# zju3dv/object_nerf

Hardware: NVIDIA H100
Metric: rays/s (higher is better)
Workload: dtype bf16

## Files before the change

object_nerf_b200/csrc/field_tc.cu:

```cuda
#include <cuda_bf16.h>

#include "encode.cuh"
#include "field_common.cuh"
#include "tc_chain.cuh"
#include "field_pe.cuh"
#include "prune.cuh"

namespace {

using namespace tc;

constexpr float kLeaky = 0.01f;

enum Epi { EPI_HIDDEN = 0, EPI_HIDDEN_RC = 1, EPI_HIDDEN_SIGMA = 2, EPI_FINAL = 3, EPI_DIR = 4 };

struct TcParams {
  FieldParams f;
  WLayer layers[MAX_LAYERS];
  int n_layers;
  uint8_t* dump;
  TrainLayout TL;
  uint32_t* diag;
#ifdef ONERF_FIELD_TIMELINE
  uint64_t* tl;
#endif
};

struct RowMeta {
  int ray, si, mute, live;
};

struct Rows {
  int row[2];
  int live[2];
  int ray[2], si[2], mute[2];
  const float* rc[2];
  int64_t tile;
#ifdef ONERF_FIELD_TIMELINE
  uint64_t* tl;
#endif
};

__device__ __forceinline__ void fragment_rows(int (&row)[2], int warp, int lane) {
  row[0] = (warp >> 2) * 64 + (warp & 3) * 16 + (lane >> 2);
  row[1] = row[0] + 8;
}

#ifdef ONERF_FIELD_TIMELINE
constexpr int TL_CTAS = 8, TL_TILES = 16, TL_SLOTS = 80;
uint64_t* g_timeline = nullptr;
__device__ __forceinline__ void tl_put(uint64_t* tl, int slot, uint64_t v) {
  asm volatile("{\n\t.reg .pred p;\n\tsetp.ne.u64 p, %0, 0;\n\t@p st.global.u64 [%1], %2;\n\t}" ::"l"(tl), "l"(tl + slot),
               "l"(v)
               : "memory");
}
__device__ __forceinline__ uint64_t* tl_record(const TcParams& P, int64_t tile, int wg, bool lead) {
  const int64_t k = (tile - blockIdx.x) / gridDim.x;
  if (!P.tl || !lead || blockIdx.x >= TL_CTAS || k >= TL_TILES) return nullptr;
  return P.tl + (((int64_t)blockIdx.x * 3 + wg) * TL_TILES + k) * TL_SLOTS;
}
#define TL_AT(tl, slot) tl_put((tl), (slot), clock64())
#define TL_PUT(tl, slot, v) tl_put((tl), (slot), (v))
#else
#define TL_AT(tl, slot)
#define TL_PUT(tl, slot, v)
#endif

__device__ __forceinline__ uint32_t leaky_bf16x2(uint32_t x) {
  __nv_bfloat162 v = *reinterpret_cast<__nv_bfloat162*>(&x);
  const __nv_bfloat162 slope = __floats2bfloat162_rn(kLeaky, kLeaky);
  v = __hmax2(v, __hmul2(v, slope));
  return *reinterpret_cast<uint32_t*>(&v);
}

template <int N>
__device__ __forceinline__ void dump_layer(const TcParams& P, const Rows& R, int slot, int mask_word0, const uint32_t* pk) {
  const int q = threadIdx.x & 3;
#pragma unroll
  for (int r = 0; r < 2; ++r) {
    const int row = R.row[r];
    uint8_t* base = P.dump + P.TL.act_off[slot] + ((size_t)R.tile * P.TL.act_atoms[slot]) * ATOM_BYTES + (size_t)row * 128 + q * 4;
#pragma unroll
    for (int j = 0; j < N / 8; ++j)
      *reinterpret_cast<uint32_t*>(base + (size_t)(j >> 3) * ATOM_BYTES + (((j & 7) ^ (row & 7)) << 4)) = pk[2 * j + r];
  }
  if (mask_word0 < 0) return;
  constexpr int CPW = N >= 128 ? 32 : 16, NW = N / CPW, BPW = CPW / 8;
  uint32_t* mrow = reinterpret_cast<uint32_t*>(P.dump + P.TL.mask_off) + ((size_t)R.tile * ONERF_MASK_WORDS + mask_word0) * 128;
#pragma unroll
  for (int w = 0; w < NW; ++w) {
#pragma unroll
    for (int r = 0; r < 2; ++r) {
      uint32_t m = 0;
#pragma unroll
      for (int jj = 0; jj < BPW; ++jj) {
        const uint32_t v = pk[2 * (w * BPW + jj) + r];
        const uint32_t bits = (((v >> 15) & 1u) ^ 1u) | ((((v >> 31) & 1u) ^ 1u) << 1);
        m |= bits << (8 * jj + 2 * q);
      }
      m |= __shfl_xor_sync(0xffffffffu, m, 1);
      m |= __shfl_xor_sync(0xffffffffu, m, 2);
      if (q == 0) mrow[w * 128 + R.row[r]] = m;
    }
  }
}

template <int N, int EPI>
__device__ __forceinline__ void epilogue(const float (&acc)[N / 2], uint32_t* pk, const float* bias, const Rows& R,
                                         int rc_base, const float* headw, float (&part)[2][4]) {
  const int q = threadIdx.x & 3;
#pragma unroll
  for (int j = 0; j < N / 8; ++j) {
    const int c = 8 * j + 2 * q;
    float2 b[2];
    if (EPI == EPI_HIDDEN_RC || EPI == EPI_DIR) {
      b[0] = __ldg(reinterpret_cast<const float2*>(R.rc[0] + rc_base + c));
      b[1] = __ldg(reinterpret_cast<const float2*>(R.rc[1] + rc_base + c));
    } else {
      b[0] = b[1] = *reinterpret_cast<const float2*>(bias + c);
    }
#pragma unroll
    for (int r = 0; r < 2; ++r) {
      float t0 = acc[4 * j + 2 * r] + b[r].x, t1 = acc[4 * j + 2 * r + 1] + b[r].y;
      uint32_t p;
      if (EPI == EPI_HIDDEN || EPI == EPI_HIDDEN_RC) {
        p = leaky_bf16x2(pack_bf16(t0, t1));
      } else if (EPI == EPI_FINAL) {
        p = pack_bf16(t0, t1);
      } else {
        t0 = fmaxf(t0, t0 * kLeaky);
        t1 = fmaxf(t1, t1 * kLeaky);
        if (EPI == EPI_HIDDEN_SIGMA) {
          const float2 w = __ldg(reinterpret_cast<const float2*>(headw + c));
          part[r][0] = fmaf(t1, w.y, fmaf(t0, w.x, part[r][0]));
        } else {
#pragma unroll
          for (int k = 0; k < 3; ++k) {
            const float2 w = __ldg(reinterpret_cast<const float2*>(headw + k * N + c));
            part[r][1 + k] = fmaf(t1, w.y, fmaf(t0, w.x, part[r][1 + k]));
          }
        }
        p = pack_bf16(t0, t1);
      }
      pk[2 * j + r] = p;
    }
  }
}

__device__ __forceinline__ float row_sum(float part) {
  part += __shfl_xor_sync(0xffffffffu, part, 1);
  part += __shfl_xor_sync(0xffffffffu, part, 2);
  return part;
}

__device__ __forceinline__ void write_heads(const FieldParams& p, const Rows& R, int branch, float (&part)[2][4],
                                            float* outp) {
  const float* Pf = reinterpret_cast<const float*>(p.packed);
  const float* hb = Pf + (branch ? p.L.orgb_b : p.L.rgb_b);
  const float sb = __ldg(Pf + (branch ? p.L.osigma_b : p.L.sigma_b));
#pragma unroll
  for (int r = 0; r < 2; ++r) {
#pragma unroll
    for (int k = 0; k < 4; ++k) part[r][k] = row_sum(part[r][k]);
    if ((threadIdx.x & 3) == 0 && R.live[r]) {
      float sg = part[r][0] + sb;
      const float cr = 1.0f / (1.0f + __expf(-(part[r][1] + __ldg(hb + 0))));
      const float cg = 1.0f / (1.0f + __expf(-(part[r][2] + __ldg(hb + 1))));
      const float cb = 1.0f / (1.0f + __expf(-(part[r][3] + __ldg(hb + 2))));
      if (R.mute[r] & (branch ? 2 : 1)) sg = -1e5f;
      reinterpret_cast<float4*>(outp)[(int64_t)R.ray[r] * p.out_stride + R.si[r]] = make_float4(cr, cg, cb, sg);
    }
  }
}

__device__ __forceinline__ void x_release(uint32_t x_free, bool on) {
  asm volatile(
      "{\n\t.reg .pred p;\n\tsetp.eq.u32 p, %1, 1;\n\t@p mbarrier.arrive.shared::cta.b64 _, [%0];\n\t}" ::"r"(x_free),
      "r"((uint32_t)on & (uint32_t)((threadIdx.x & 31) == 0))
      : "memory");
}

template <int N, int NX, int NH, int EPI, bool DUMP>
__device__ __forceinline__ void run_layer(const TcParams& P, const Rows& R, Ring& ring, uint32_t sXw, float (&acc)[N / 2],
                                          const uint32_t* hin, uint32_t* hout, const float* bias, int rc_base,
                                          const float* headw, float (&part)[2][4], int slot, int mask_word0,
                                          uint32_t x_free = 0, bool free_x = false) {
  TL_AT(R.tl, 3 * slot);
  mma_layer<N, NX, NH>(acc, hin, sXw, ring);
  if constexpr (NX > 0) x_release(x_free, free_x);
  TL_AT(R.tl, 3 * slot + 1);
#ifdef ONERF_FIELD_TIMELINE
  TL_PUT(R.tl, 55 + slot, ring.full_wait);
  ring.full_wait = 0;
#endif
  epilogue<N, EPI>(acc, hout, bias, R, rc_base, headw, part);
  if (DUMP) dump_layer<N>(P, R, slot, mask_word0, hout);
  TL_AT(R.tl, 3 * slot + 2);
}

template <int XS, bool DUMP>
__device__ __forceinline__ void scene_trunk(const TcParams& P, const Rows& R, Ring& ring, uint32_t sXw, float (&acc)[128],
                                            uint32_t (&h)[64], const float* bias_tab, float (&part)[2][4],
                                            uint32_t x_free) {
  const float* sw = reinterpret_cast<const float*>(P.f.packed) + P.f.L.sigma_w;
  run_layer<256, XS, 0, EPI_HIDDEN, DUMP>(P, R, ring, sXw, acc, h, h, bias_tab + G_S0 * 256, 0, nullptr, part, 1,
                                          onerf_mask_word0(1), x_free, false);
#pragma unroll 1
  for (int l = 1; l < 4; ++l)
    run_layer<256, 0, 8, EPI_HIDDEN, DUMP>(P, R, ring, sXw, acc, h, h, bias_tab + (G_S0 + l) * 256, 0, nullptr, part,
                                           1 + l, onerf_mask_word0(1 + l));
  run_layer<256, XS, 8, EPI_HIDDEN, DUMP>(P, R, ring, sXw, acc, h, h, bias_tab + G_S4 * 256, 0, nullptr, part, 5,
                                          onerf_mask_word0(5), x_free, true);
#pragma unroll 1
  for (int l = 5; l < 7; ++l)
    run_layer<256, 0, 8, EPI_HIDDEN, DUMP>(P, R, ring, sXw, acc, h, h, bias_tab + (G_S0 + l) * 256, 0, nullptr, part,
                                           1 + l, onerf_mask_word0(1 + l));
  run_layer<256, 0, 8, EPI_HIDDEN_SIGMA, DUMP>(P, R, ring, sXw, acc, h, h, bias_tab + G_S7 * 256, 0, sw, part, 8,
                                               onerf_mask_word0(8));
}

constexpr int NUM_ENCODER = 3 * 32;

__device__ __forceinline__ void prefetch_l2(const void* ptr) {
  asm volatile("prefetch.global.L2 [%0];" ::"l"(ptr));
}

__device__ __forceinline__ void prefetch_rows(const void* base, int64_t pitch, int64_t bytes0, int nbytes, int r0,
                                              int r1, int et) {
  const int lines = (nbytes + 127) >> 7;
  for (int i = et; i < (r1 - r0 + 1) * lines; i += NUM_ENCODER)
    prefetch_l2(reinterpret_cast<const char*>(base) + (r0 + i / lines) * pitch + bytes0 + (int64_t)(i % lines) * 128);
}

__device__ __forceinline__ void voxel_encode_job(const GridView& g, uint32_t sX, int row, int cq, float x, float y,
                                                 float z, uint32_t x_free, uint32_t parity, uint32_t* diag) {
  if (cq < 3) {
    float f[8];
    if (cq == 0) voxel_trilinear<0, 8, false>(g, x, y, z, f);
    else if (cq == 1) voxel_trilinear<8, 8, false>(g, x, y, z, f);
    else voxel_trilinear<16, 8, false>(g, x, y, z, f);
    mbar_wait(x_free, parity, diag);
    pe8_to_chunks(sX, row, cq < 2 ? cq : 34, cq < 2 ? 2 : 1, f);
  } else if (cq == 3) {
    mbar_wait(x_free, parity, diag);
    pe_xyz_to_chunks(sX, row, 26, x, y, z);
    st_chunk(a_chunk_addr(sX, row, 47), 0u, 0u, 0u, 0u);
  }
}

template <bool VOXEL>
__device__ __forceinline__ void encoder_loop(const TcParams& P, uint32_t sX, RowMeta* meta, uint32_t x_full,
                                             uint32_t x_free, int64_t n_tiles, int64_t total) {
  const FieldParams& p = P.f;
  const int et = threadIdx.x - NUM_CONSUMER - 32;
  constexpr int JOBS = VOXEL ? 4 * TM : TM;
  uint32_t it = 0;
  for (int64_t tile = blockIdx.x; tile < n_tiles; tile += gridDim.x, ++it) {
#ifdef ONERF_FIELD_TIMELINE
    uint64_t* tl = tl_record(P, tile, 2, et == 0);
#endif
    TL_AT(tl, 0);
    {
      const int64_t e0 = tile * TM, e1 = min(e0 + TM, total) - 1;
      prefetch_rows(p.ray_const, ONERF_RAY_CONST_FLOATS * 4, 0, ONERF_RAY_CONST_FLOATS * 4, (int)(e0 / p.S),
                    (int)(e1 / p.S), et);
      const int64_t n0 = e0 + (int64_t)gridDim.x * TM, n1 = min(n0 + TM, total) - 1;
      if (n0 < total) {
        prefetch_rows(p.rays, 32, 0, 32, (int)(n0 / p.S), (int)(n1 / p.S), et);
        prefetch_rows(p.z, p.z_stride * 4, 0, p.S * 4, (int)(n0 / p.S), (int)(n1 / p.S), et);
      }
    }
#pragma unroll 1
    for (int job = et; job < JOBS; job += NUM_ENCODER) {
      const int row = job & (TM - 1), cq = job / TM;
      const int64_t e = tile * TM + row;
      const bool live = e < total;
      const int ray = live ? (int)(e / p.S) : 0;
      const int si = live ? (int)(e - (int64_t)ray * p.S) : 0;
      const float* rr = p.rays + (int64_t)ray * 8;
      const float zz = live ? __ldg(p.z + (int64_t)ray * p.z_stride + si) : 0.0f;
      float x = fmaf(__ldg(rr + 3), zz, __ldg(rr + 0));
      float y = fmaf(__ldg(rr + 4), zz, __ldg(rr + 1));
      float z = fmaf(__ldg(rr + 5), zz, __ldg(rr + 2));
      if (p.xyz && live) {
        const float* qq = p.xyz + ((int64_t)ray * p.S + si) * 3;
        x = __ldg(qq); y = __ldg(qq + 1); z = __ldg(qq + 2);
      }
      if (!live) { x = 0.f; y = 0.f; z = 0.f; }
      if (cq == 0) {
        int mute = 0;
        if (live && p.mute_zero_rays && __ldg(p.z + (int64_t)ray * p.z_stride + (p.S - 1)) == 0.0f) mute = 3;
        if (live && mute == 0 && p.n_boxes > 0 && point_in_boxes(p.boxes, p.n_boxes, x, y, z)) mute = 1;
        mbar_wait(x_free, (it & 1) ^ 1, P.diag);
        meta[row] = RowMeta{ray, si, mute, live ? 1 : 0};
      }
      if (VOXEL) {
        voxel_encode_job(load_grid_view(p.grid), sX, row, cq, x, y, z, x_free, (it & 1) ^ 1, P.diag);
      } else if (cq == 0) {
        mbar_wait(x_free, (it & 1) ^ 1, P.diag);
        pe_xyz_to_chunks(sX, row, 0, x, y, z);
      }
    }
    mbar_wait(x_free, (it & 1) ^ 1, P.diag);
    TL_AT(tl, 1);
    fence_async_smem();
    mbar_arrive(x_full);
    TL_AT(tl, 2);
  }
}

struct FieldSmem {
  uint32_t sB, sBias, sMeta, sBar, x_full, x_free, bytes;
};
__host__ __device__ constexpr FieldSmem field_smem(int x_atoms, bool has_meta) {
  FieldSmem s{};
  s.sB = x_atoms * ATOM_BYTES;
  s.sBias = s.sB + NSTAGE * STAGE_BYTES;
  s.sMeta = s.sBias + G_COUNT * 256 * 4;
  s.sBar = s.sMeta + (has_meta ? TM * (uint32_t)sizeof(RowMeta) : 0u);
  s.x_full = s.sBar + 16 * NSTAGE;
  s.x_free = s.x_full + 8;
  s.bytes = 1024 + s.x_free + 8;
  return s;
}

__device__ __forceinline__ Ring cta_prologue(const FieldSmem& S, const TcParams& P, uint32_t sX, float* bias_tab) {
  const FieldParams& p = P.f;
  const float* Pf = reinterpret_cast<const float*>(p.packed);
  Ring ring{sX + S.sB, sX + S.sBar, sX + S.sBar + 8 * NSTAGE, 0u, 0u, P.diag};
  if (threadIdx.x == 0) {
    mbar_init(sX + S.x_full, NUM_ENCODER);
    mbar_init(sX + S.x_free, NUM_CONSUMER / 32);
    ring_init_bars(ring.full, ring.empty);
  }
  for (int i = threadIdx.x; i < G_COUNT * 256; i += NUM_THREADS) {
    const int g = i >> 8, c = i & 255;
    bias_tab[i] = (c < p.L.g[g].N) ? __ldg(Pf + p.L.g[g].bias_off + c) : 0.0f;
  }
  __syncthreads();
  return ring;
}

struct CodeLoop {
  int n;
  int64_t rc_stride, obj_stride;
};

template <bool VOXEL, bool DUMP, bool MULTI>
__device__ __forceinline__ void field_tc_body(const TcParams& P, const CodeLoop& cl) {
  extern __shared__ __align__(1024) uint8_t smem_raw[];
  const FieldParams& p = P.f;
  const int warp = threadIdx.x >> 5, lane = threadIdx.x & 31;
  constexpr int X_ATOMS = VOXEL ? 6 : 1;
  constexpr int XS = VOXEL ? 9 : 2, XO = VOXEL ? 12 : 2;
  constexpr FieldSmem S = field_smem(X_ATOMS, true);
  const uint32_t sX = (smem_u32(smem_raw) + 1023u) & ~1023u;
  uint8_t* gen_base = smem_raw + (sX - smem_u32(smem_raw));
  float* bias_tab = reinterpret_cast<float*>(gen_base + S.sBias);
  RowMeta* meta = reinterpret_cast<RowMeta*>(gen_base + S.sMeta);
  const uint32_t x_full = sX + S.x_full, x_free = sX + S.x_free;
  const float* Pf = reinterpret_cast<const float*>(p.packed);
  Ring ring = cta_prologue(S, P, sX, bias_tab);

  const int64_t total = (int64_t)field_rays(p) * p.S;
  const int64_t n_tiles = (total + TM - 1) / TM;

  if (warp >= PRODUCER_WARP) {
    setmaxnreg_dec<PRODUCER_REGS>();
    if (warp == PRODUCER_WARP) {
      if constexpr (MULTI)
        tc_producer_loop(P.layers, P.n_layers, reinterpret_cast<const uint8_t*>(p.packed), ring, n_tiles,
                         G_ODIR - G_O0 + 1, cl.n);
      else
        tc_producer_loop(P.layers, P.n_layers, reinterpret_cast<const uint8_t*>(p.packed), ring, n_tiles);
    } else
      encoder_loop<VOXEL>(P, sX, meta, x_full, x_free, n_tiles, total);
    return;
  }
  setmaxnreg_inc<CONSUMER_REGS>();

  const int wg = warp >> 2, tid = threadIdx.x & 127;
  const uint32_t sXw = sX + (uint32_t)wg * 64u * 128u;
  const bool free_after_o2 = !p.want_scene;
  Rows R;
  fragment_rows(R.row, warp, lane);
  uint32_t it = 0;
  for (int64_t tile = blockIdx.x; tile < n_tiles; tile += gridDim.x, ++it) {
    R.tile = tile;
#ifdef ONERF_FIELD_TIMELINE
    R.tl = tl_record(P, tile, wg, tid == 0);
#endif
    TL_AT(R.tl, 0);
    mbar_wait(x_full, it & 1, P.diag);
    TL_AT(R.tl, 1);
    if (DUMP) {
#pragma unroll 1
      for (int a = 0; a < X_ATOMS; ++a) {
        const uint4* src = reinterpret_cast<const uint4*>(gen_base + (size_t)a * ATOM_BYTES + (size_t)wg * 8192);
        uint4* dst = reinterpret_cast<uint4*>(P.dump + P.TL.act_off[0] + ((size_t)tile * X_ATOMS + a) * ATOM_BYTES + (size_t)wg * 8192);
        for (int i = tid; i < 512; i += 128) dst[i] = src[i];
      }
    }
#pragma unroll
    for (int r = 0; r < 2; ++r) {
      const RowMeta m = meta[R.row[r]];
      R.live[r] = m.live; R.ray[r] = m.ray; R.si[r] = m.si; R.mute[r] = m.mute;
      R.rc[r] = p.ray_const + (int64_t)m.ray * ONERF_RAY_CONST_FLOATS;
    }
    TL_AT(R.tl, 2);

    if (p.want_object) {
      const float* rc0[2] = {R.rc[0], R.rc[1]};
      for (int c = 0; c < (MULTI ? cl.n : 1); ++c) {
        if constexpr (MULTI) {
          R.rc[0] = rc0[0] + c * cl.rc_stride;
          R.rc[1] = rc0[1] + c * cl.rc_stride;
        }
        float acc[64];
        uint32_t h[32];
        float part[2][4] = {};
        run_layer<128, XO, 0, EPI_HIDDEN_RC, DUMP>(P, R, ring, sXw, acc, h, h, nullptr, RC_OL0, nullptr, part, 11,
                                                   onerf_mask_word0(11), x_free, false);
        run_layer<128, 0, 4, EPI_HIDDEN, DUMP>(P, R, ring, sXw, acc, h, h, bias_tab + G_O1 * 256, 0, nullptr, part, 12,
                                               onerf_mask_word0(12));
        run_layer<128, XO, 4, EPI_HIDDEN_RC, DUMP>(P, R, ring, sXw, acc, h, h, nullptr, RC_OL2, nullptr, part, 13,
                                                   onerf_mask_word0(13), x_free, MULTI ? free_after_o2 && c == cl.n - 1 : free_after_o2);
        run_layer<128, 0, 4, EPI_HIDDEN_SIGMA, DUMP>(P, R, ring, sXw, acc, h, h, bias_tab + G_O3 * 256, 0,
                                                     Pf + p.L.osigma_w, part, 14, onerf_mask_word0(14));
        run_layer<128, 0, 4, EPI_FINAL, DUMP>(P, R, ring, sXw, acc, h, h, bias_tab + G_OFIN * 256, 0, nullptr, part, 15, -1);
        float accd[32];
        uint32_t hd[16];
        run_layer<64, 0, 4, EPI_DIR, DUMP>(P, R, ring, sXw, accd, h, hd, nullptr, RC_ODIR, Pf + p.L.orgb_w, part, 16,
                                           onerf_mask_word0(16));
        write_heads(p, R, 1, part, MULTI ? p.obj_out + c * cl.obj_stride : p.obj_out);
      }
      if constexpr (MULTI) {
        R.rc[0] = rc0[0];
        R.rc[1] = rc0[1];
      }
    }
    if (p.want_scene) {
      float acc[128];
      uint32_t h[64];
      float part[2][4] = {};
      scene_trunk<XS, DUMP>(P, R, ring, sXw, acc, h, bias_tab, part, x_free);
      run_layer<256, 0, 8, EPI_FINAL, DUMP>(P, R, ring, sXw, acc, h, h, bias_tab + G_SFIN * 256, 0, nullptr, part, 9, -1);
      float accd[64];
      uint32_t hd[32];
      run_layer<128, 0, 8, EPI_DIR, DUMP>(P, R, ring, sXw, accd, h, hd, nullptr, RC_SDIR, Pf + p.L.rgb_w, part, 10,
                                          onerf_mask_word0(10));
      write_heads(p, R, 0, part, p.scene_out);
    }
    TL_AT(R.tl, 51);
    TL_AT(R.tl, 52);
  }
}

template <bool VOXEL, bool DUMP>
__global__ void __launch_bounds__(NUM_THREADS, 1) field_tc_kernel(const __grid_constant__ TcParams P) {
  field_tc_body<VOXEL, DUMP, false>(P, CodeLoop{1, 0, 0});
}

struct MultiTcParams {
  TcParams t;
  CodeLoop codes;
};

template <bool VOXEL>
__global__ void __launch_bounds__(NUM_THREADS, 1) field_tc_multi_kernel(const __grid_constant__ MultiTcParams Q) {
  field_tc_body<VOXEL, false, true>(Q.t, Q.codes);
}

struct PruneTcParams {
  TcParams t;
  PruneSource src;
  int64_t cell_begin, n_cells;
  uint32_t* max_alpha;
};
constexpr int kPruneTilesPerVoxel = kPruneSamples / TM;
static_assert(kPruneSamples % TM == 0, "a tile must lie inside one voxel");

__device__ __forceinline__ void prune_encoder_loop(const PruneTcParams& Q, uint32_t sX, uint32_t x_full, uint32_t x_free,
                                                   int64_t n_tiles) {
  const int et = threadIdx.x - NUM_CONSUMER - 32;
  const GridView g = load_grid_view(Q.t.f.grid);
  uint32_t it = 0;
  for (int64_t tile = blockIdx.x; tile < n_tiles; tile += gridDim.x, ++it) {
    const int64_t k = Q.cell_begin + tile / kPruneTilesPerVoxel;
    const int s0 = (int)(tile % kPruneTilesPerVoxel) * TM;
#pragma unroll 1
    for (int job = et; job < 4 * TM; job += NUM_ENCODER) {
      const int row = job & (TM - 1);
      float p[3];
      prune_point(Q.src, g, k, s0 + row, p);
      voxel_encode_job(g, sX, row, job / TM, p[0], p[1], p[2], x_free, (it & 1) ^ 1, Q.t.diag);
    }
    mbar_wait(x_free, (it & 1) ^ 1, Q.t.diag);
    fence_async_smem();
    mbar_arrive(x_full);
  }
}

__global__ void __launch_bounds__(NUM_THREADS, 1) prune_tc_kernel(const __grid_constant__ PruneTcParams Q) {
  extern __shared__ __align__(1024) uint8_t smem_raw[];
  const TcParams& P = Q.t;
  const FieldParams& p = P.f;
  const int warp = threadIdx.x >> 5, lane = threadIdx.x & 31;
  constexpr FieldSmem S = field_smem(6, false);
  const uint32_t sX = (smem_u32(smem_raw) + 1023u) & ~1023u;
  float* bias_tab = reinterpret_cast<float*>(smem_raw + (sX - smem_u32(smem_raw)) + S.sBias);
  const uint32_t x_full = sX + S.x_full, x_free = sX + S.x_free;
  Ring ring = cta_prologue(S, P, sX, bias_tab);

  const int64_t n_tiles = Q.n_cells * kPruneTilesPerVoxel;
  if (warp >= PRODUCER_WARP) {
    setmaxnreg_dec<PRODUCER_REGS>();
    if (warp == PRODUCER_WARP)
      tc_producer_loop(P.layers, P.n_layers, reinterpret_cast<const uint8_t*>(p.packed), ring, n_tiles);
    else
      prune_encoder_loop(Q, sX, x_full, x_free, n_tiles);
    return;
  }
  setmaxnreg_inc<CONSUMER_REGS>();

  const uint32_t sXw = sX + (uint32_t)(warp >> 2) * 64u * 128u;
  const float sb = __ldg(reinterpret_cast<const float*>(p.packed) + p.L.sigma_b);
  Rows R;
  fragment_rows(R.row, warp, lane);
#ifdef ONERF_FIELD_TIMELINE
  R.tl = nullptr;
#endif
  uint32_t it = 0;
  for (int64_t tile = blockIdx.x; tile < n_tiles; tile += gridDim.x, ++it) {
    R.tile = tile;
    mbar_wait(x_full, it & 1, P.diag);
    float acc[128];
    uint32_t h[64];
    float part[2][4] = {};
    scene_trunk<9, false>(P, R, ring, sXw, acc, h, bias_tab, part, x_free);
    float m = 0.0f;
#pragma unroll
    for (int r = 0; r < 2; ++r) m = fmaxf(m, prune_alpha(row_sum(part[r][0]) + sb));
#pragma unroll
    for (int o = 16; o > 0; o >>= 1) m = fmaxf(m, __shfl_xor_sync(0xffffffffu, m, o));
    asm volatile("{\n\t.reg .pred p;\n\tsetp.eq.u32 p, %2, 0;\n\t@p red.global.max.u32 [%0], %1;\n\t}" ::"l"(
                     Q.max_alpha + tile / kPruneTilesPerVoxel),
                 "r"(__float_as_uint(m)), "r"(lane)
                 : "memory");
  }
}

void add_layers(TcParams& P, int g0, int g1) {
  for (int g = g0; g <= g1; ++g) P.layers[P.n_layers++] = WLayer{P.f.L.g[g].img_off, P.f.L.g[g].N, P.f.L.g[g].K / 32};
}

template <class Params>
int launch_persistent(onerf_ctx* ctx, void (*kernel)(Params), const Params& P, int64_t tiles, size_t smem,
                      cudaStream_t stream) {
  const int blocks = (int)(tiles < ctx->num_sms ? tiles : ctx->num_sms);
  ONERF_CUDA(cudaFuncSetAttribute(kernel, cudaFuncAttributeMaxDynamicSharedMemorySize, (int)smem));
  kernel<<<blocks, NUM_THREADS, smem, stream>>>(P);
  ONERF_LAUNCH_CHECK(ctx);
  return ONERF_OK;
}

}

int onerf_launch_field_bf16(onerf_ctx* ctx, const FieldParams& fp, cudaStream_t stream) {
  TcParams P;
  memset(&P, 0, sizeof(P));
  P.f = fp;
  if (fp.want_object) add_layers(P, G_O0, G_ODIR);
  if (fp.want_scene) add_layers(P, G_S0, G_SDIR);
  P.diag = ctx->tc_diag;
#ifdef ONERF_FIELD_TIMELINE
  P.tl = g_timeline;
#endif
  const bool voxel = fp.L.use_voxel, train = fp.train_ws != nullptr;
  const int64_t total = (int64_t)fp.n_rays * fp.S;
  if (train) {
    P.dump = reinterpret_cast<uint8_t*>(fp.train_ws);
    P.TL = onerf_make_train_layout(voxel, total);
  }
  auto* kernel = voxel ? (train ? field_tc_kernel<true, true> : field_tc_kernel<true, false>)
                       : (train ? field_tc_kernel<false, true> : field_tc_kernel<false, false>);
  return launch_persistent(ctx, kernel, P, (total + TM - 1) / TM, field_smem(voxel ? 6 : 1, true).bytes, stream);
}

int onerf_launch_field_bf16_codes(onerf_ctx* ctx, const FieldParams& fp, int n_codes, int64_t rc_stride,
                                  int64_t obj_stride, cudaStream_t stream) {
  ONERF_CHECK_ARG(fp.want_object && !fp.train_ws && n_codes >= 1, "a multi-code launch is an object-branch inference");
  MultiTcParams Q;
  memset(&Q, 0, sizeof(Q));
  Q.t.f = fp;
  add_layers(Q.t, G_O0, G_ODIR);
  if (fp.want_scene) add_layers(Q.t, G_S0, G_SDIR);
  Q.t.diag = ctx->tc_diag;
#ifdef ONERF_FIELD_TIMELINE
  Q.t.tl = g_timeline;
#endif
  Q.codes = CodeLoop{n_codes, rc_stride, obj_stride};
  const bool voxel = fp.L.use_voxel;
  const int64_t total = (int64_t)fp.n_rays * fp.S;
  return launch_persistent(ctx, voxel ? field_tc_multi_kernel<true> : field_tc_multi_kernel<false>, Q,
                           (total + TM - 1) / TM, field_smem(voxel ? 6 : 1, true).bytes, stream);
}

int onerf_launch_prune_bf16(onerf_ctx* ctx, const FieldParams& fp, const PruneSource& src, int64_t cell_begin,
                            int64_t n_cells, float* max_alpha, cudaStream_t stream) {
  PruneTcParams Q;
  memset(&Q, 0, sizeof(Q));
  Q.t.f = fp;
  add_layers(Q.t, G_S0, G_S7);
  Q.t.diag = ctx->tc_diag;
  Q.src = src;
  Q.cell_begin = cell_begin;
  Q.n_cells = n_cells;
  Q.max_alpha = reinterpret_cast<uint32_t*>(max_alpha);
  return launch_persistent(ctx, prune_tc_kernel, Q, n_cells * kPruneTilesPerVoxel,
                           field_smem(6, false).bytes, stream);
}

#ifdef ONERF_FIELD_TIMELINE
extern "C" void onerf_field_timeline(void* buf) { g_timeline = static_cast<uint64_t*>(buf); }
#endif
```

Baseline: 1.547 million.

## Stage head weights in smem, preload ray constants, double-buffer row metadata

Copies the sigma/rgb head weights for both branches into the shared-memory bias table so the epilogue reads them from shared rather than global memory. Per-ray constants for the first fragment row are loaded before the MMA loop so their latency overlaps the matrix work. When S is a multiple of 64, both fragment rows belong to the same ray and the second load is skipped. Row metadata becomes double-buffered per tile parity and is read on demand instead of being cached in registers, which frees registers but adds shared-memory loads and smem footprint.

New measurement: 1.590 million, median of 6. +2.8%, better.

```diff
diff --git a/object_nerf_b200/csrc/field_tc.cu b/object_nerf_b200/csrc/field_tc.cu
--- a/object_nerf_b200/csrc/field_tc.cu
+++ b/object_nerf_b200/csrc/field_tc.cu
@@ -32,9 +32,9 @@
 
 struct Rows {
   int row[2];
-  int live[2];
-  int ray[2], si[2], mute[2];
-  const float* rc[2];
+  bool one_ray;
+  const RowMeta* meta;
+  const float* rc;
   int64_t tile;
 #ifdef ONERF_FIELD_TIMELINE
   uint64_t* tl;
@@ -105,17 +105,39 @@
   }
 }
 
+__host__ __device__ constexpr bool has_rc(int epi) { return epi == EPI_HIDDEN_RC || epi == EPI_DIR; }
+
+constexpr int HW_SIGMA = G_COUNT * 256, HW_RGB = HW_SIGMA + 256, HW_OSIGMA = HW_RGB + 3 * 128,
+              HW_ORGB = HW_OSIGMA + 128, TAB_FLOATS = HW_ORGB + 3 * 64;
+static_assert(TAB_FLOATS % 4 == 0, "RowMeta after the table stays 16-byte aligned");
+
+__device__ __forceinline__ const float* rc_row(const Rows& R, int row, int rc_base) {
+  return R.rc + (int64_t)R.meta[row].ray * ONERF_RAY_CONST_FLOATS + rc_base;
+}
+
 template <int N, int EPI>
+__device__ __forceinline__ void rc_preload(const Rows& R, int rc_base, float2 (&rc0)[N / 8]) {
+  if constexpr (has_rc(EPI)) {
+    const float* src = rc_row(R, R.row[0], rc_base) + 2 * (threadIdx.x & 3);
+#pragma unroll
+    for (int j = 0; j < N / 8; ++j) rc0[j] = __ldg(reinterpret_cast<const float2*>(src + 8 * j));
+  }
+}
+
+template <int N, int EPI, bool ONE_RAY = false>
 __device__ __forceinline__ void epilogue(const float (&acc)[N / 2], uint32_t* pk, const float* bias, const Rows& R,
-                                         int rc_base, const float* headw, float (&part)[2][4]) {
+                                         int rc_base, const float2 (&rc0)[N / 8], const float* headw,
+                                         float (&part)[2][4]) {
   const int q = threadIdx.x & 3;
+  const float* rc1 = nullptr;
+  if constexpr (has_rc(EPI) && !ONE_RAY) rc1 = rc_row(R, R.row[1], rc_base);
 #pragma unroll
   for (int j = 0; j < N / 8; ++j) {
     const int c = 8 * j + 2 * q;
     float2 b[2];
-    if (EPI == EPI_HIDDEN_RC || EPI == EPI_DIR) {
-      b[0] = __ldg(reinterpret_cast<const float2*>(R.rc[0] + rc_base + c));
-      b[1] = __ldg(reinterpret_cast<const float2*>(R.rc[1] + rc_base + c));
+    if constexpr (has_rc(EPI)) {
+      b[0] = rc0[j];
+      b[1] = ONE_RAY ? rc0[j] : __ldg(reinterpret_cast<const float2*>(rc1 + c));
     } else {
       b[0] = b[1] = *reinterpret_cast<const float2*>(bias + c);
     }
@@ -131,12 +153,12 @@
         t0 = fmaxf(t0, t0 * kLeaky);
         t1 = fmaxf(t1, t1 * kLeaky);
         if (EPI == EPI_HIDDEN_SIGMA) {
-          const float2 w = __ldg(reinterpret_cast<const float2*>(headw + c));
+          const float2 w = *reinterpret_cast<const float2*>(headw + c);
           part[r][0] = fmaf(t1, w.y, fmaf(t0, w.x, part[r][0]));
         } else {
 #pragma unroll
           for (int k = 0; k < 3; ++k) {
-            const float2 w = __ldg(reinterpret_cast<const float2*>(headw + k * N + c));
+            const float2 w = *reinterpret_cast<const float2*>(headw + k * N + c);
             part[r][1 + k] = fmaf(t1, w.y, fmaf(t0, w.x, part[r][1 + k]));
           }
         }
@@ -162,13 +184,14 @@
   for (int r = 0; r < 2; ++r) {
 #pragma unroll
     for (int k = 0; k < 4; ++k) part[r][k] = row_sum(part[r][k]);
-    if ((threadIdx.x & 3) == 0 && R.live[r]) {
+    const RowMeta m = R.meta[R.row[r]];
+    if ((threadIdx.x & 3) == 0 && m.live) {
       float sg = part[r][0] + sb;
       const float cr = 1.0f / (1.0f + __expf(-(part[r][1] + __ldg(hb + 0))));
       const float cg = 1.0f / (1.0f + __expf(-(part[r][2] + __ldg(hb + 1))));
       const float cb = 1.0f / (1.0f + __expf(-(part[r][3] + __ldg(hb + 2))));
-      if (R.mute[r] & (branch ? 2 : 1)) sg = -1e5f;
-      reinterpret_cast<float4*>(outp)[(int64_t)R.ray[r] * p.out_stride + R.si[r]] = make_float4(cr, cg, cb, sg);
+      if (m.mute & (branch ? 2 : 1)) sg = -1e5f;
+      reinterpret_cast<float4*>(outp)[(int64_t)m.ray * p.out_stride + m.si] = make_float4(cr, cg, cb, sg);
     }
   }
 }
@@ -186,6 +209,8 @@
                                           const float* headw, float (&part)[2][4], int slot, int mask_word0,
                                           uint32_t x_free = 0, bool free_x = false) {
   TL_AT(R.tl, 3 * slot);
+  float2 rc0[N / 8];
+  rc_preload<N, EPI>(R, rc_base, rc0);
   mma_layer<N, NX, NH>(acc, hin, sXw, ring);
   if constexpr (NX > 0) x_release(x_free, free_x);
   TL_AT(R.tl, 3 * slot + 1);
@@ -193,7 +218,10 @@
   TL_PUT(R.tl, 55 + slot, ring.full_wait);
   ring.full_wait = 0;
 #endif
-  epilogue<N, EPI>(acc, hout, bias, R, rc_base, headw, part);
+  if (has_rc(EPI) && R.one_ray)
+    epilogue<N, EPI, true>(acc, hout, bias, R, rc_base, rc0, headw, part);
+  else
+    epilogue<N, EPI>(acc, hout, bias, R, rc_base, rc0, headw, part);
   if (DUMP) dump_layer<N>(P, R, slot, mask_word0, hout);
   TL_AT(R.tl, 3 * slot + 2);
 }
@@ -202,7 +230,7 @@
 __device__ __forceinline__ void scene_trunk(const TcParams& P, const Rows& R, Ring& ring, uint32_t sXw, float (&acc)[128],
                                             uint32_t (&h)[64], const float* bias_tab, float (&part)[2][4],
                                             uint32_t x_free) {
-  const float* sw = reinterpret_cast<const float*>(P.f.packed) + P.f.L.sigma_w;
+  const float* sw = bias_tab + HW_SIGMA;
   run_layer<256, XS, 0, EPI_HIDDEN, DUMP>(P, R, ring, sXw, acc, h, h, bias_tab + G_S0 * 256, 0, nullptr, part, 1,
                                           onerf_mask_word0(1), x_free, false);
 #pragma unroll 1
@@ -292,7 +320,7 @@
         if (live && p.mute_zero_rays && __ldg(p.z + (int64_t)ray * p.z_stride + (p.S - 1)) == 0.0f) mute = 3;
         if (live && mute == 0 && p.n_boxes > 0 && point_in_boxes(p.boxes, p.n_boxes, x, y, z)) mute = 1;
         mbar_wait(x_free, (it & 1) ^ 1, P.diag);
-        meta[row] = RowMeta{ray, si, mute, live ? 1 : 0};
+        meta[(it & 1) * TM + row] = RowMeta{ray, si, mute, live ? 1 : 0};
       }
       if (VOXEL) {
         voxel_encode_job(load_grid_view(p.grid), sX, row, cq, x, y, z, x_free, (it & 1) ^ 1, P.diag);
@@ -316,8 +344,8 @@
   FieldSmem s{};
   s.sB = x_atoms * ATOM_BYTES;
   s.sBias = s.sB + NSTAGE * STAGE_BYTES;
-  s.sMeta = s.sBias + G_COUNT * 256 * 4;
-  s.sBar = s.sMeta + (has_meta ? TM * (uint32_t)sizeof(RowMeta) : 0u);
+  s.sMeta = s.sBias + TAB_FLOATS * 4;
+  s.sBar = s.sMeta + (has_meta ? 2 * TM * (uint32_t)sizeof(RowMeta) : 0u);
   s.x_full = s.sBar + 16 * NSTAGE;
   s.x_free = s.x_full + 8;
   s.bytes = 1024 + s.x_free + 8;
@@ -336,6 +364,12 @@
   for (int i = threadIdx.x; i < G_COUNT * 256; i += NUM_THREADS) {
     const int g = i >> 8, c = i & 255;
     bias_tab[i] = (c < p.L.g[g].N) ? __ldg(Pf + p.L.g[g].bias_off + c) : 0.0f;
+  }
+  for (int i = HW_SIGMA + threadIdx.x; i < TAB_FLOATS; i += NUM_THREADS) {
+    const int64_t src = i < HW_RGB ? p.L.sigma_w + (i - HW_SIGMA)
+                        : i < HW_OSIGMA ? p.L.rgb_w + (i - HW_RGB)
+                        : i < HW_ORGB ? p.L.osigma_w + (i - HW_OSIGMA) : p.L.orgb_w + (i - HW_ORGB);
+    bias_tab[i] = __ldg(Pf + src);
   }
   __syncthreads();
   return ring;
@@ -384,9 +418,12 @@
   const bool free_after_o2 = !p.want_scene;
   Rows R;
   fragment_rows(R.row, warp, lane);
+  R.one_ray = p.S % 64 == 0;
   uint32_t it = 0;
   for (int64_t tile = blockIdx.x; tile < n_tiles; tile += gridDim.x, ++it) {
     R.tile = tile;
+    R.meta = meta + (it & 1) * TM;
+    R.rc = p.ray_const;
 #ifdef ONERF_FIELD_TIMELINE
     R.tl = tl_record(P, tile, wg, tid == 0);
 #endif
@@ -401,21 +438,11 @@
         for (int i = tid; i < 512; i += 128) dst[i] = src[i];
       }
     }
-#pragma unroll
-    for (int r = 0; r < 2; ++r) {
-      const RowMeta m = meta[R.row[r]];
-      R.live[r] = m.live; R.ray[r] = m.ray; R.si[r] = m.si; R.mute[r] = m.mute;
-      R.rc[r] = p.ray_const + (int64_t)m.ray * ONERF_RAY_CONST_FLOATS;
-    }
     TL_AT(R.tl, 2);
 
     if (p.want_object) {
-      const float* rc0[2] = {R.rc[0], R.rc[1]};
       for (int c = 0; c < (MULTI ? cl.n : 1); ++c) {
-        if constexpr (MULTI) {
-          R.rc[0] = rc0[0] + c * cl.rc_stride;
-          R.rc[1] = rc0[1] + c * cl.rc_stride;
-        }
+        if constexpr (MULTI) R.rc = p.ray_const + c * cl.rc_stride;
         float acc[64];
         uint32_t h[32];
         float part[2][4] = {};
@@ -426,18 +453,15 @@
         run_layer<128, XO, 4, EPI_HIDDEN_RC, DUMP>(P, R, ring, sXw, acc, h, h, nullptr, RC_OL2, nullptr, part, 13,
                                                    onerf_mask_word0(13), x_free, MULTI ? free_after_o2 && c == cl.n - 1 : free_after_o2);
         run_layer<128, 0, 4, EPI_HIDDEN_SIGMA, DUMP>(P, R, ring, sXw, acc, h, h, bias_tab + G_O3 * 256, 0,
-                                                     Pf + p.L.osigma_w, part, 14, onerf_mask_word0(14));
+                                                     bias_tab + HW_OSIGMA, part, 14, onerf_mask_word0(14));
         run_layer<128, 0, 4, EPI_FINAL, DUMP>(P, R, ring, sXw, acc, h, h, bias_tab + G_OFIN * 256, 0, nullptr, part, 15, -1);
         float accd[32];
         uint32_t hd[16];
-        run_layer<64, 0, 4, EPI_DIR, DUMP>(P, R, ring, sXw, accd, h, hd, nullptr, RC_ODIR, Pf + p.L.orgb_w, part, 16,
+        run_layer<64, 0, 4, EPI_DIR, DUMP>(P, R, ring, sXw, accd, h, hd, nullptr, RC_ODIR, bias_tab + HW_ORGB, part, 16,
                                            onerf_mask_word0(16));
         write_heads(p, R, 1, part, MULTI ? p.obj_out + c * cl.obj_stride : p.obj_out);
       }
-      if constexpr (MULTI) {
-        R.rc[0] = rc0[0];
-        R.rc[1] = rc0[1];
-      }
+      if constexpr (MULTI) R.rc = p.ray_const;
     }
     if (p.want_scene) {
       float acc[128];
@@ -447,7 +471,7 @@
       run_layer<256, 0, 8, EPI_FINAL, DUMP>(P, R, ring, sXw, acc, h, h, bias_tab + G_SFIN * 256, 0, nullptr, part, 9, -1);
       float accd[64];
       uint32_t hd[32];
-      run_layer<128, 0, 8, EPI_DIR, DUMP>(P, R, ring, sXw, accd, h, hd, nullptr, RC_SDIR, Pf + p.L.rgb_w, part, 10,
+      run_layer<128, 0, 8, EPI_DIR, DUMP>(P, R, ring, sXw, accd, h, hd, nullptr, RC_SDIR, bias_tab + HW_RGB, part, 10,
                                           onerf_mask_word0(10));
       write_heads(p, R, 0, part, p.scene_out);
     }
```
